# cipherflow-fhe/lattisense

Measured on AMD Instinct MI355X. Metric: ckks_hmult_relin_rescale_throughput, higher is better.
Workload: dtype u64

## Files before the change

include/lattisense_amd.h:

```cpp
#ifndef LATTISENSE_AMD_H
#define LATTISENSE_AMD_H
#include <stddef.h>
#include <stdint.h>

#ifdef __cplusplus
extern "C" {
#endif

typedef struct lsa_context_st* lsa_context;
typedef struct lsa_key_st* lsa_key;

enum { LSA_OK = 0, LSA_ERR_ARG = 1, LSA_ERR_NO_DEVICE = 2, LSA_ERR_HIP = 3, LSA_ERR_INTERNAL = 4 };
enum { LSA_ALGO_BFV = 0, LSA_ALGO_CKKS = 1 };

const char* lsa_last_error(void);
const char* lsa_version(void);
const char* lsa_build_flags(void);

int lsa_context_create(int algo, int n, const uint64_t* q, int nq, const uint64_t* p, int np, uint64_t t,
                       int device, lsa_context* out);
int lsa_context_destroy(lsa_context ctx);
int lsa_context_moduli(lsa_context ctx, uint64_t* out, int capacity, int* count);

int lsa_malloc(lsa_context ctx, void** dptr, size_t bytes);
// ... 70 lines not shown
                          const uint64_t* const* pts, const long long* spts, const uint64_t* partial, long long spartial,
                          uint64_t* out, int batch, long long sout, void* stream);
int lsa_bfv_rotate_mac_plain_mul(lsa_context ctx, int level, const uint64_t* in, int n, const uint64_t* galois_elements,
                                 const lsa_key* glk, const uint64_t* const* pts, const long long* spts, const uint64_t* partial,
                                 long long spartial, uint64_t* out, int batch, long long sin, long long sout, void* stream);
int lsa_bfv_rescale(lsa_context ctx, int level, int polys, const uint64_t* in, uint64_t* out, int batch,
                    long long stride_in, long long stride_out, void* stream);
int lsa_bfv_mult_relin(lsa_context ctx, int level, const uint64_t* a, const uint64_t* b, lsa_key rlk,
                       uint64_t* out, int batch, long long stride_a, long long stride_b, long long stride_out,
                       void* stream);

int lsa_set_tile_batch(lsa_context ctx, int tile_batch);
int lsa_set_fp64_ntt(lsa_context ctx, int enable);
int lsa_set_dual_stream(lsa_context ctx, int enable);
int lsa_set_fuse_tails(lsa_context ctx, int enable);
int lsa_set_ntt_chunk_mib(lsa_context ctx, int mib);
int lsa_ckks_rotate_many(lsa_context ctx, int level, const uint64_t* in, int n_rot, const uint64_t* galois_elements,
                         const lsa_key* glk, uint64_t* const* outs, int batch, long long sin, long long sout, void* stream);
int lsa_bfv_rotate_many(lsa_context ctx, int level, const uint64_t* in, int n_rot, const uint64_t* galois_elements,
                        const lsa_key* glk, uint64_t* const* outs, int batch, long long sin, long long sout, void* stream);

typedef struct lsa_bootstrap_st* lsa_bootstrap;
int lsa_bootstrap_create(lsa_context ctx, int cts_depth, int stc_depth, int k, int double_angle, double message_ratio,
                         double in_scale, double out_scale, int log_slots, void* stream, lsa_bootstrap* out);
int lsa_bootstrap_create_ex(lsa_context ctx, int cts_depth, int stc_depth, int k, int double_angle, double message_ratio,
                            double in_scale, double out_scale, int log_slots, int sine_deg, int arcsine_deg, void* stream,
                            lsa_bootstrap* out);
int lsa_bootstrap_evalmod_constants(lsa_bootstrap b, int* n_cheb, double* cheb, int* n_asin, double* asin_coef);
void lsa_bootstrap_destroy(lsa_bootstrap b);
int lsa_bootstrap_info(lsa_bootstrap b, int* out_level, double* out_scale, int* n_galois, int* n_matrices, int* n_cts,
// ... 54 lines not shown
```

lattisense_amd/_native.py:

```python
import ctypes
import importlib.util
import os

_HERE = os.path.dirname(os.path.abspath(__file__))
LIB_PATH = os.environ.get("LSA_NATIVE_LIB") or os.path.join(_HERE, "liblattisense_amd.so")

_lib = None

c_u64p = ctypes.POINTER(ctypes.c_uint64)
c_ll = ctypes.c_longlong
c_vp = ctypes.c_void_p
c_int = ctypes.c_int


class LsaError(RuntimeError):
    def __init__(self, code, msg):
        super().__init__("lattisense_amd error %d: %s" % (code, msg))
        self.code = code


def _preload_hip_runtime():
    spec = importlib.util.find_spec("torch")
    if spec is not None and spec.origin:
        p = os.path.join(os.path.dirname(spec.origin), "lib", "libamdhip64.so")
# ... 46 lines not shown
    "lsa_ckks_mult_const": (c_int, [c_vp, c_int, c_vp, c_ll, ctypes.c_double, ctypes.c_double, ctypes.c_double, c_vp, c_ll, c_int,
                                    c_int, c_vp]),
    "lsa_ckks_add_const": (c_int, [c_vp, c_int, c_vp, c_ll, ctypes.c_double, ctypes.c_double, ctypes.c_double, c_vp, c_ll, c_int,
                                   c_vp]),
    "lsa_ckks_affine_const": (c_int, [c_vp, c_int, c_vp, c_ll, ctypes.c_double, ctypes.c_double, ctypes.c_double, ctypes.c_double,
                                      ctypes.c_double, ctypes.c_double, c_vp, c_ll, c_int, c_int, c_vp]),
    "lsa_bfv_mult": (c_int, [c_vp, c_int, c_vp, c_vp, c_vp, c_int, c_ll, c_ll, c_ll, c_vp]),
    "lsa_bfv_relin": (c_int, [c_vp, c_int, c_vp, c_vp, c_vp, c_int, c_ll, c_ll, c_vp]),
    "lsa_bfv_rotate": (c_int, [c_vp, c_int, c_vp, ctypes.c_uint64, c_vp, c_vp, c_int, c_ll, c_ll, c_vp]),
    "lsa_bfv_rescale": (c_int, [c_vp, c_int, c_int, c_vp, c_vp, c_int, c_ll, c_ll, c_vp]),
    "lsa_bfv_mult_relin": (c_int, [c_vp, c_int, c_vp, c_vp, c_vp, c_vp, c_int, c_ll, c_ll, c_ll, c_vp]),
    "lsa_set_tile_batch": (c_int, [c_vp, c_int]),
    "lsa_set_fp64_ntt": (c_int, [c_vp, c_int]),
    "lsa_set_dual_stream": (c_int, [c_vp, c_int]),
    "lsa_set_fuse_tails": (c_int, [c_vp, c_int]),
    "lsa_set_ntt_chunk_mib": (c_int, [c_vp, c_int]),
    "lsa_debug_set_ntt_stamps": (c_int, [c_vp, c_vp]),
    "lsa_debug_baseconv_plans": (c_int, [c_vp, c_int, ctypes.POINTER(c_int), ctypes.POINTER(c_int), ctypes.POINTER(c_int),
                                         ctypes.POINTER(c_int)]),
    "lsa_debug_key_switch_fused": (c_int, [c_vp, c_int, c_vp, ctypes.POINTER(c_int)]),
    "lsa_ckks_rotate_many": (c_int, [c_vp, c_int, c_vp, c_int, c_u64p, ctypes.POINTER(c_vp), ctypes.POINTER(c_vp), c_int,
                                     ctypes.c_longlong, ctypes.c_longlong, c_vp]),
    "lsa_bfv_rotate_many": (c_int, [c_vp, c_int, c_vp, c_int, c_u64p, ctypes.POINTER(c_vp), ctypes.POINTER(c_vp), c_int,
                                    ctypes.c_longlong, ctypes.c_longlong, c_vp]),
    "lsa_bfv_mult_plain_mul": (c_int, [c_vp, c_int, c_vp, c_vp, c_vp, c_int, c_ll, c_ll, c_ll, c_vp]),
    "lsa_bfv_mac_plain_mul": (c_int, [c_vp, c_int, c_int, ctypes.POINTER(c_vp), ctypes.POINTER(c_ll), ctypes.POINTER(c_vp),
                                      ctypes.POINTER(c_ll), c_vp, c_ll, c_vp, c_int, c_ll, c_vp]),
    "lsa_bfv_rotate_mac_plain_mul": (c_int, [c_vp, c_int, c_vp, c_int, c_u64p, ctypes.POINTER(c_vp), ctypes.POINTER(c_vp),
                                             ctypes.POINTER(c_ll), c_vp, c_ll, c_vp, c_int, c_ll, c_ll, c_vp]),
    "lsa_bootstrap_create": (c_int, [c_vp, c_int, c_int, c_int, c_int, ctypes.c_double, ctypes.c_double, ctypes.c_double, c_int,
# ... 77 lines not shown
```

lattisense_amd/csrc/build_flags.h:

```cpp
#pragma once

#if (defined(LSA_NTT_DIAG_NO_TWIDDLE_LOADS) || defined(LSA_NTT_DIAG_COPY_ONLY) || defined(LSA_NTT_DIAG_COMPUTE_ONLY) || defined(LSA_NTT_DIAG_TW8) || \
     defined(LSA_KS_DIAG_NO_MATH) || defined(LSA_KS_DIAG_NO_STORE) || defined(LSA_BC_DIAG_NO_MATH) || defined(LSA_BC_DIAG_NO_STORE)) && \
    !defined(LSA_DIAG_BUILD)
#error "wrong-result diagnostic switches need -DLSA_DIAG_BUILD (use lattisense_amd.build --variant: it adds the flag and renames the library)"
#endif

#define LSA_BF_STR2(x) #x
#define LSA_BF_STR(x) LSA_BF_STR2(x)

#define LSA_BUILD_FLAGS_TEXT_1 ""
#ifdef LSA_DIAG_BUILD
#define LSA_BF_DIAG " LSA_DIAG_BUILD"
#else
#define LSA_BF_DIAG ""
#endif
#ifdef LSA_NTT_DIAG_NO_TWIDDLE_LOADS
#define LSA_BF_A " LSA_NTT_DIAG_NO_TWIDDLE_LOADS"
#else
#define LSA_BF_A ""
#endif
#ifdef LSA_NTT_DIAG_COPY_ONLY
#define LSA_BF_B " LSA_NTT_DIAG_COPY_ONLY"
#else
// ... 127 lines not shown
#if defined(LSA_KSMAC_WAVES_FP) && LSA_KSMAC_WAVES_FP != 2
#define LSA_BF_AE " LSA_KSMAC_WAVES_FP=" LSA_BF_STR(LSA_KSMAC_WAVES_FP)
#else
#define LSA_BF_AE ""
#endif
#if defined(LSA_KSMAC_CHUNK) && LSA_KSMAC_CHUNK != 4
#define LSA_BF_AF " LSA_KSMAC_CHUNK=" LSA_BF_STR(LSA_KSMAC_CHUNK)
#else
#define LSA_BF_AF ""
#endif
#ifdef LSA_NTT_DIAG_TW8
#define LSA_BF_AD " LSA_NTT_DIAG_TW8"
#else
#define LSA_BF_AD ""
#endif
#ifdef LSA_VARIANT_NAME
#define LSA_BF_V " variant=" LSA_BF_STR(LSA_VARIANT_NAME)
#else
#define LSA_BF_V ""
#endif
#ifdef LSA_AB_SWITCH
#define LSA_BF_W " LSA_AB_SWITCH=" LSA_BF_STR(LSA_AB_SWITCH)
#else
#define LSA_BF_W ""
#endif

#define LSA_BUILD_FLAGS_TEXT                                                                                              \
    LSA_BF_DIAG LSA_BF_A LSA_BF_B LSA_BF_C LSA_BF_D LSA_BF_E LSA_BF_F LSA_BF_G LSA_BF_H LSA_BF_I LSA_BF_J LSA_BF_K LSA_BF_L \
        LSA_BF_M LSA_BF_N LSA_BF_O LSA_BF_P LSA_BF_Q LSA_BF_R LSA_BF_S LSA_BF_T LSA_BF_U LSA_BF_V LSA_BF_W LSA_BF_X LSA_BF_Y LSA_BF_Z LSA_BF_AA LSA_BF_AB LSA_BF_AC LSA_BF_AD LSA_BF_AE LSA_BF_AF
```

lattisense_amd/csrc/c_api.hip:

```cpp
#include "build_flags.h"
#include "linear_transform.h"
#include "poly_eval.h"
#include "lsa_internal.h"

namespace lsa {
const char* kernels_build_flags();
const char* context_build_flags();
}

using namespace lsa;

struct lsa_context_st {
    Context ctx;
    lsa_context_st(int algo, int n, const u64* q, int nq, const u64* p, int np, u64 t, int dev)
        : ctx(algo, n, q, nq, p, np, t, dev) {}
};
struct lsa_key_st {
    Key key;
    double* fp_owned = nullptr;
};

template <typename F>
static int guard(F&& f) {
    try {
// ... 354 lines not shown

int lsa_profile_read_primary(lsa_context ctx, int kind, double* total_bytes_primary) {
    return guard([&] {
        Context& c = C(ctx);
        LSA_REQUIRE(kind >= 0 && kind < LSA_PROF_KINDS && total_bytes_primary, "bad argument");
        double by = 0;
        for (auto& sm : c.prof_samples)
            if (sm.kid == kind) by += sm.bytes_primary;
        *total_bytes_primary = by;
    });
}

int lsa_set_fuse_tails(lsa_context ctx, int enable) {
    return guard([&] { C(ctx).fuse_tails = enable ? 1 : 0; });
}
int lsa_set_dual_stream(lsa_context ctx, int enable) {
    return guard([&] { C(ctx).dual_stream = enable ? 1 : 0; });
}
int lsa_debug_set_ntt_stamps(lsa_context ctx, void* device_buffer) {
    return guard([&] { C(ctx).ntt_diag = static_cast<unsigned long long*>(device_buffer); });
}
int lsa_debug_baseconv_plans(lsa_context ctx, int capacity, int* count, int* ns, int* nd, int* split) {
    return guard([&] {
        Context& c = C(ctx);
        LSA_REQUIRE(count != nullptr && (capacity == 0 || (ns && nd && split)), "null argument");
        std::lock_guard<std::mutex> lk(c.mu);
        *count = (int)c.bconv.size();
        int i = 0;
        for (auto& kv : c.bconv) {
            if (i >= capacity) break;
// ... 382 lines not shown
```

lattisense_amd/csrc/emu_ntt.cpp:

```cpp
#define LSA_EMULATE 1
#include <cstddef>
#include <vector>
#include "ntt_plan.h"
#include "ntt_r16.h"
#include <array>
#include "tables.h"

template <int NT>
static void emu_block(const NttPassArgs& a, const NttBlockCtx& bc, u64* lds) {
    for (int t = 0; t < NT; t++) ntt_phase_load<true, NT, true>(a, bc, t, lds);
    int rho[4];
    const int np = ntt_split(a.mu, rho);
    if (!a.inverse) {
        int sig = 0;
        for (int i = 0; i < np; i++) {
            for (int t = 0; t < NT; t++) ntt_phase_sub_dyn<NT>(a, bc, t, lds, sig, rho[i]);
            sig += rho[i];
        }
    } else {
        int sig = a.mu;
        for (int i = np - 1; i >= 0; i--) {
            sig -= rho[i];
            for (int t = 0; t < NT; t++) ntt_phase_sub_dyn<NT>(a, bc, t, lds, sig, rho[i]);
        }
    }
    for (int t = 0; t < NT; t++) ntt_phase_store<true, NT>(a, bc, t, lds);
}

template <int PASS, int MU>
static void emu_block_r16(const NttPassArgs& a, const NttBlockCtx& bc, u64* lds) {
    std::vector<std::array<u64, 16>> regs(LSA_R16_THREADS);
    for (int phase = 0; phase < 3; phase++)
        for (int t = 0; t < LSA_R16_THREADS; t++) {
            u64(&v)[16] = *reinterpret_cast<u64(*)[16]>(regs[t].data());
            r16_phase<PASS, 3 | 16, MU>(a, bc, t, lds, phase, v);
        }
}

static void emu_block_r8x3(const NttPassArgs& a, const NttBlockCtx& bc, u64* lds) {
    std::vector<std::array<u64, 16>> regs(LSA_R16_THREADS);
    for (int phase = 0; phase < 4; phase++)
        for (int t = 0; t < LSA_R16_THREADS; t++) {
            u64(&v)[16] = *reinterpret_cast<u64(*)[16]>(regs[t].data());
            r8x3_phase<3 | 16>(a, bc, t, lds, phase, v);
        }
}

static int emu_ntt(int n, const u64* moduli, int nmod, u64* data, int batch, long long batch_stride, int rows,
                   const unsigned char* mod_of, int period, int inverse, int tau_max, int allow_fp64, const u64* pa, const u64* pb) {
    const int row_inner = (allow_fp64 >> 1) & 1;
    const bool r16 = (allow_fp64 >> 2) & 1;
    allow_fp64 &= 1;
    lsa::HostTables T;
    T.build(n, std::vector<u64>(moduli, moduli + nmod));
    NttPlan plan = make_ntt_plan(T.logn, tau_max);
    std::vector<u64> tw_i(T.psi.size());
    std::vector<double> tw_d(T.psi_d.size());
    for (int m = 0; m < nmod; m++) {
        const size_t o = (size_t)m * n;
        ntt_permute_twiddles(plan, T.logn, (inverse ? T.psiinv : T.psi).data() + 2 * o, tw_i.data() + 2 * o, 2, false);
        ntt_permute_twiddles(plan, T.logn, (inverse ? T.psiinv_d : T.psi_d).data() + o, tw_d.data() + o, 1, true);
    }
    NttPassArgs a{};
    a.src = data;
// ... 9 lines not shown
    a.scaled = T.scale_d.data();
    a.allow_fp64 = allow_fp64;
    a.period = period;
    a.row0 = 0;
    a.row_step = 1;
    a.row_inner = row_inner;
    for (int i = 0; i < period; i++) a.mod_of[i] = mod_of[i];
    if (pa) {
        a.fz_pro = 3;
        a.fz_limbs = rows;
        a.fz_a = pa;
        a.fz_b = pb;
        a.fz_a_stride = a.fz_b_stride = batch_stride;
        a.fz_a_rpp = a.fz_b_rpp = rows;
    }
    int launch_rows = 0;
    for (int r = 0; r < rows; r++)
        if (mod_of[r % period] != LSA_ROW_SKIP) a.row_tbl[launch_rows++] = (unsigned short)r;
    a.compact = 1;
    a.rows = launch_rows;
    for (int step = 0; step < plan.npass; step++) {
        int k = inverse ? plan.npass - 1 - step : step;
        ntt_fill_pass(a, plan, T.logn, k, inverse);
        a.fz_first = step == 0;
        a.fp_raw_out = plan.npass == 2 && step == 0;
        a.fp_raw_in = plan.npass == 2 && step == 1;
        std::vector<u64> lds(lds_words(a.tau));
        long long nblocks = (long long)batch * launch_rows * (1 << (a.logn - a.tau));
        for (long long bid = 0; bid < nblocks; bid++) {
            NttBlockCtx bc = ntt_decode_block(a, bid);
            if (bc.mod == LSA_ROW_SKIP) continue;
            if (r16 && ntt_r16_shape_ok(a, plan.npass)) {
                if (a.mu == 9) emu_block_r8x3(a, bc, lds.data());
                else if (a.lambda && a.mu == 8) emu_block_r16<0, 8>(a, bc, lds.data());
                else if (a.lambda) emu_block_r16<0, 7>(a, bc, lds.data());
                else if (a.mu == 8) emu_block_r16<1, 8>(a, bc, lds.data());
                else emu_block_r16<1, 7>(a, bc, lds.data());
            } else if (a.tau <= 12) emu_block<LSA_NTT_THREADS>(a, bc, lds.data());
            else if (a.tau == 13) emu_block<512>(a, bc, lds.data());
            else emu_block<1024>(a, bc, lds.data());
        }
    }
    return 0;
}

extern "C" int lsa_emu_ntt(int n, const u64* moduli, int nmod, u64* data, int batch, long long batch_stride, int rows,
                           const unsigned char* mod_of, int period, int inverse, int tau_max, int allow_fp64) {
    return emu_ntt(n, moduli, nmod, data, batch, batch_stride, rows, mod_of, period, inverse, tau_max, allow_fp64, nullptr, nullptr);
}

extern "C" int lsa_emu_intt_prod(int n, const u64* moduli, int nmod, const u64* pa, const u64* pb, u64* out, int batch,
                                 long long batch_stride, int rows, const unsigned char* mod_of, int period, int tau_max,
                                 int allow_fp64) {
    if (!pa || !pb) return -1;
    return emu_ntt(n, moduli, nmod, out, batch, batch_stride, rows, mod_of, period, 1, tau_max, allow_fp64, pa, pb);
}
```

lattisense_amd/csrc/kernels.hip:

```cpp
#include <atomic>
#include <cstdlib>

#include "build_flags.h"
#include "lsa_internal.h"
#include "ntt_r16.h"
#include "plain_ops.h"
#include "poly_lincomb.h"
#include "tensor_sum.h"

namespace lsa {

const char* kernels_build_flags() { return LSA_BUILD_FLAGS_TEXT; }

static constexpr int TPB = 256;

#ifndef LSA_NTT_WAVES
#define LSA_NTT_WAVES 4
#endif

#if defined(LSA_NTT_DIAG_STAMPS)
#define LSA_STAMP(k)                                                                               \
    do {                                                                                           \
        if (a.diag && threadIdx.x == 0 && blockIdx.x < 8192) a.diag[blockIdx.x * 8 + (k)] = __builtin_amdgcn_s_memtime(); \
    } while (0)
// ... 127 lines not shown
    const bool pro = fused && a.fz_pro && a.fz_first, epi = fused && a.fz_epi && a.final_reduce;
    if (pro && a.fz_pro == 3) return 16;
    if (epi && a.fz_epi == 3) return 4;
    if (epi && a.fz_epi == 4) return 8;
    return (pro ? 1 : 0) | (epi ? 2 : 0);
}
template <int FZ>
static auto ntt_r16_second_pass(int mu) {
    return mu == 9 ? &k_ntt_r8x3<FZ> : mu == 8 ? &k_ntt_r16<1, FZ, 8> : &k_ntt_r16<1, FZ, 7>;
}
static bool ntt_launch_r16(const NttPassArgs& a, int npass, bool fused, long long nblocks, hipStream_t s) {
    if (!sw::ntt_r16() || !ntt_r16_shape_ok(a, npass)) return false;
    const int fz = ntt_pass_fz(a, fused);
    void (*k)(NttPassArgs) = nullptr;
    if (a.lambda) {
        if (fz == 1 && a.mu == 8 && sw::r16_pro()) k = &k_ntt_r16<0, 1, 8>;
        else if (fz == 0) k = a.mu == 8 ? &k_ntt_r16<0, 0, 8> : &k_ntt_r16<0, 0, 7>;
    } else if (a.mu != 9 || sw::ntt_r8x3()) {
        switch (fz) {
            case 0: k = ntt_r16_second_pass<0>(a.mu); break;
            case 2: k = ntt_r16_second_pass<2>(a.mu); break;
            case 4: k = ntt_r16_second_pass<4>(a.mu); break;
            case 8: k = ntt_r16_second_pass<8>(a.mu); break;
            case 16: k = a.inverse ? ntt_r16_second_pass<16>(a.mu) : nullptr; break;
        }
    }
    if (!k) return false;
    hipLaunchKernelGGL(k, dim3((unsigned)nblocks), dim3(LSA_R16_THREADS), (size_t)LSA_R16_LDS_WORDS * sizeof(u64), s, a);
    LSA_HIP(hipGetLastError());
    return true;
}
// ... 211 lines not shown
                const RowMap& rm, bool inverse, hipStream_t s, const NttFusion* fz, int passes) {
    if (batch <= 0 || rows <= 0) return;
    LSA_REQUIRE(rm.period >= 1 && rm.period <= LSA_MAX_PERIOD, "ntt: bad row-map period");
    NttPassArgs a{};
    a.batch = batch;
    a.rows = rows;
    a.mods = c.d_mods;
    a.scale = c.d_scale;
    a.diag = c.ntt_diag;
    a.scaled = c.d_scale_d;
    a.allow_fp64 = c.fp64_ntt;
    if (fz) {
        LSA_REQUIRE(!inverse || (fz->pro == 3 && !fz->epi), "inverse transforms take the product prologue only");
        LSA_REQUIRE(fz->pro != 3 || (inverse && !fz->epi && fz->a && fz->b && fz->limbs >= 1 && (passes & 1)),
                    "product prologue: an inverse transform from its first pass, two operands, no epilogue");
        a.fz_epi = fz->epi;
        a.fz_pro = fz->pro;
        a.fz_limbs = fz->limbs;
        a.fz_base_polys = fz->base_polys;
        a.fz_ql_mod = fz->ql_mod;
        a.fz_a = fz->a;
        a.fz_a_stride = fz->a_stride;
        a.fz_a_rpp = fz->a_rpp;
        a.fz_base = fz->base;
        a.fz_base_stride = fz->base_stride;
        a.fz_base_rpp = fz->base_rpp;
        a.fz_k = fz->k;
        a.fz_out = fz->out;
        a.fz_out_stride = fz->out_stride;
        a.fz_out_rpp = fz->out_rpp;
// ... 50 lines not shown
    if (passes != 3) wide = false;
    if (fz && fz->pro == 3) wide = false;
    const NttPlan& plan = wide ? c.plan_wide : c.plan;
    a.tw = wide ? (inverse ? c.d_psiinv_w : c.d_psi_w) : (inverse ? c.d_psiinv : c.d_psi);
    a.twd = wide ? (inverse ? c.d_psiinv_d_w : c.d_psi_d_w) : (inverse ? c.d_psiinv_d : c.d_psi_d);
    {
        bool any_fp = false, any_int = false;
        for (int r = 0; r < rows; r++) {
            const unsigned char m = rm.mod_of[(rm.row0 + r * rm.row_step) % rm.period];
            if (m == LSA_ROW_SKIP) continue;
            const bool fp = c.fp_engine(m);
            any_fp |= fp;
            any_int |= !fp;
        }
        a.row_inner = any_fp && any_int;
    }
    int chunk = batch;
    if (plan.npass > 1 && c.ntt_chunk_mib > 0) {
        const double per_item = 8.0 * c.n * std::max(active_rows, 1);
        chunk = (int)std::max(1.0, std::min((double)batch, c.ntt_chunk_mib * 1048576.0 / per_item));
    }
    for (int b0 = 0; b0 < batch; b0 += chunk) {
        const int nb = std::min(chunk, batch - b0);
        a.batch = nb;
        if (fz && fz->epi == 3) {
            a.fz_a = fz->a + (long long)b0 * fz->a_stride;
            a.fz_base = fz->base ? fz->base + (long long)b0 * fz->base_stride : nullptr;
            a.fz_out = fz->out + (long long)b0 * fz->out_stride;
        }
        if (fz && fz->epi == 4) {
            a.fz_a = fz->a + (long long)b0 * fz->a_stride;
            a.fz_base = fz->base ? fz->base + (long long)b0 * fz->base_stride : nullptr;
            a.fz_pt = fz->pt + (long long)b0 * fz->pt_stride;
            a.fz_out = fz->out + (long long)b0 * fz->out_stride;
        }
        if (fz && fz->pro == 3) {
            a.fz_a = fz->a + (long long)b0 * fz->a_stride;
            a.fz_b = fz->b + (long long)b0 * fz->b_stride;
        }
        bool first = true;
        for (int step = 0; step < plan.npass; step++) {
            if (plan.npass == 2 && !((passes >> step) & 1)) continue;
            a.fz_first = first ? 1 : 0;
            first = false;
            const int k = inverse ? plan.npass - 1 - step : step;
            ntt_fill_pass(a, plan, c.logn, k, inverse ? 1 : 0);
            a.fp_raw_out = plan.npass == 2 && step == 0 && c.fp_raw;
            a.fp_raw_in = plan.npass == 2 && step == 1 && c.fp_raw;
            LSA_REQUIRE(!(a.fz_first && a.fz_pro && a.fp_raw_in), "ntt: a fused prologue reads canonical inputs, never a raw hand-off");
            a.src = (step == 0 ? src + (long long)b0 * src_stride : dst + (long long)b0 * dst_stride);
// ... 1929 lines not shown
```

lattisense_amd/csrc/lsa_internal.h:

```cpp
#pragma once
#include <hip/hip_runtime.h>
#include <cstdint>
#include <map>
#include <memory>
#include <mutex>
#include <stdexcept>
#include <string>
#include <vector>

#include "../../include/lattisense_amd.h"
#include "ntt_plan.h"
#include "plain_ops.h"
#include "switches.h"
#include "tables.h"

namespace lsa {

struct Error : std::runtime_error {
    int code;
    Error(int c, const std::string& m) : std::runtime_error(m), code(c) {}
};

void set_last_error(const std::string& m);

// ... 57 lines not shown
    int wide_mode = 2;
    ModDev* d_mods = nullptr;
    u64* d_psi = nullptr;
    u64* d_psiinv = nullptr;
    u64* d_scale = nullptr;
    double* d_psi_d = nullptr;
    double* d_psiinv_d = nullptr;
    u64* d_psi_w = nullptr;
    u64* d_psiinv_w = nullptr;
    double* d_psi_d_w = nullptr;
    double* d_psiinv_d_w = nullptr;
    double* d_scale_d = nullptr;
    int fp64_ntt = 1;
    int tile_batch = 0;
    int fp_raw = 1;
    int fuse_tails = 1;
    int dual_stream = 0;
    hipStream_t aux_stream = nullptr;
    hipEvent_t ev_fork = nullptr, ev_join = nullptr;
    void fork_aux(hipStream_t s);
    void join_aux(hipStream_t s);
    unsigned long long* ntt_diag = nullptr;
    int ntt_chunk_mib = 0;

    struct ProfSample {
        hipEvent_t e0, e1;
        int kid;
        double bytes;
        double bytes_primary;
    };
// ... 300 lines not shown
```

lattisense_amd/csrc/ntt_core.h:

```cpp
#pragma once
#include "modarith.h"

#ifndef LSA_NTT_THREADS
#define LSA_NTT_THREADS 256
#endif
#define LSA_MAX_PERIOD 192
#if defined(LSA_EMULATE)
#include <cstdio>
#include <cstdlib>
#define LSA_EMU_CHECK(c) do { if (!(c)) { std::fprintf(stderr, "ntt replay: range invariant violated: %s (%s:%d)\n", #c, __FILE__, __LINE__); std::abort(); } } while (0)
#else
#define LSA_EMU_CHECK(c) do { } while (0)
#endif
#define LSA_ROW_SKIP 0xFF
#define LSA_FP64_MAX_BITS 47
#ifndef LSA_NTT_MAX_RHO
#define LSA_NTT_MAX_RHO 4
#endif

struct NttPassArgs {
    const u64* src;
    u64* dst;
    long long src_stride;
    long long dst_stride;
// ... 212 lines not shown
LSA_HD u64 double_to_u52(double r) { return d_to_bits(r + 4503599627370496.0) & 0x000FFFFFFFFFFFFFull; }
LSA_HD double fp_modmul(double v, double w, double q, double qinv) {
    const double h = v * w;
    const double l = __builtin_fma(v, w, -h);
    const double c = __builtin_rint(h * qinv);
    const double d = __builtin_fma(-c, q, h);
    return d + l;
}
LSA_HD double fp_reduce(double x, double q, double qinv) { return __builtin_fma(-__builtin_rint(x * qinv), q, x); }

#define LSA_NTT_STAGE_PAIRS 8
#ifndef LSA_NTT_HEAD_ROUNDS
#define LSA_NTT_HEAD_ROUNDS 2
#endif
struct NttLoadFix {
    bool head, add, fp, near, raw, fp_lift;
    u64 ql, h, hq;
    double hd, qld;
    ModDev mi;
};
LSA_HD u64 ntt_load_fix(const NttLoadFix& f, u64 v, u64 t) {
    if (f.fp_lift) {
        const double td = u52_to_double(t);
        const double r = td > f.hd ? td - f.qld : td;
        return d_to_bits(f.add ? u52_to_double(v) + r : r);
    }
    if (f.head) {
        const u64 c = add_mod(t, f.h, f.ql);
        const u64 lift = sub_mod(f.near ? csub(c, f.mi.q) : reduce_u64(c, f.mi), f.hq, f.mi.q);
        v = f.add ? add_mod(v, lift, f.mi.q) : lift;
    }
    if (f.fp && !f.raw) v = d_to_bits(u52_to_double(v));
    return v;
}
template <bool FZ>
LSA_HD NttLoadFix ntt_make_load_fix(const NttPassArgs& a, const NttBlockCtx& bc, const u64*& g, const u64*& gl) {
    g = a.src + bc.base_src;
    gl = g;
    NttLoadFix f;
    f.head = FZ && (a.fz_pro == 1 || a.fz_pro == 2) && a.fz_first;
    f.add = f.head && a.fz_pro == 2;
    f.fp = bc.fp != 0;
    f.raw = f.fp && a.fp_raw_in;
    LSA_EMU_CHECK(!(a.fz_pro && a.fz_first && a.fp_raw_in));
    f.mi = a.mods[bc.mod];
    f.ql = f.h = f.hq = 0;
    f.hd = f.qld = 0.0;
    f.near = f.fp_lift = false;
    if (f.head) {
        gl = a.fz_last + (long long)bc.b * a.fz_last_stride + ((long long)(bc.row / a.fz_limbs) * a.fz_last_rpp << a.logn);
        if (!f.add) g = gl;
        f.ql = a.mods[a.fz_ql_mod].q;
        f.h = (f.ql - 1) >> 1;
        f.hq = reduce_u64(f.h, f.mi);
        f.near = f.ql <= 2 * f.mi.q;
        f.fp_lift = f.fp && (f.ql >> 48) == 0;
        f.hd = (double)f.h;
        f.qld = (double)f.ql;
    }
    return f;
}
struct NttProdFix {
    const u64* pa;
// ... 52 lines not shown
            lds[lds_addr(2 * i)] = ntt_prod_fix(pf, pf.pa[x], pf.pb[x]);
            lds[lds_addr(2 * i + 1)] = ntt_prod_fix(pf, pf.pa[x + 1], pf.pb[x + 1]);
        }
        return;
    }
    const NttLoadFix f = ntt_make_load_fix<FZ>(a, bc, g, gl);
    const NttTileMap tm = ntt_tile_map(a, bc.tile);
    if (half == LSA_NTT_STAGE_PAIRS * NT && !f.add) {
        NttLoadFix f1 = f;
        f1.add = false;
        u64 st[2 * LSA_NTT_STAGE_PAIRS];
#pragma unroll
        for (int p = 0; p < LSA_NTT_STAGE_PAIRS; p++) {
            const int x = ntt_tile_index(tm, 2 * (tid + p * NT));
            ntt_load_data_pair(g + x, st[2 * p], st[2 * p + 1]);
        }
#pragma unroll
        for (int p = 0; p < LSA_NTT_STAGE_PAIRS; p++) {
            const int l = 2 * (tid + p * NT);
            lds[lds_addr(l)] = ntt_load_fix(f1, st[2 * p], st[2 * p]);
            lds[lds_addr(l + 1)] = ntt_load_fix(f1, st[2 * p + 1], st[2 * p + 1]);
        }
        return;
    }
    if (half == LSA_NTT_STAGE_PAIRS * NT) {
        constexpr int CH = LSA_NTT_STAGE_PAIRS / LSA_NTT_HEAD_ROUNDS;
#pragma unroll 1
        for (int p0 = 0; p0 < LSA_NTT_STAGE_PAIRS; p0 += CH) {
            u64 st[2 * CH], sl[2 * CH];
#pragma unroll
// ... 635 lines not shown
```

lattisense_amd/csrc/ntt_r16.h:

```cpp
#pragma once
#include "ntt_core.h"

#define LSA_R16_THREADS 256
#define LSA_R16_LDS_WORDS (272 * 16)

LSA_HD bool ntt_r16_shape_ok(const NttPassArgs& a, int npass) {
    if (npass != 2 || a.tau != 12) return false;
    if (a.mu == 9) return a.s_lo == a.logn - 9 && a.lambda == 0;
    if (a.mu != 8 && a.mu != 7) return false;
    return (a.s_lo == 0 && a.lambda == 12 - a.mu) || (a.s_lo == a.logn - a.mu && a.lambda == 0);
}

template <int PASS, int MU>
LSA_HD int r16_lds(int k, int i) {
    const int p = i + (i >> 4);
    return PASS == 0 ? (p << (12 - MU)) + k : k * ((1 << MU) + (1 << (MU - 4))) + p;
}
template <int PASS, int MU>
LSA_HD long long r16_x(const NttPassArgs& a, int tile, int k, int i) {
    return PASS == 0 ? ((long long)tile << (12 - MU)) + ((long long)i << (a.logn - MU)) + k : ((long long)tile << 12) + (k << MU) + i;
}
template <int MU, int IMAGE>
LSA_HD int r16_pt(int i, int e) {
    return IMAGE == 0 ? i + (e << (MU - 4)) : 16 * i + e;
// ... 67 lines not shown
LSA_HD void r16_lane(int tid, int& k, int& i) {
    if (PASS == 0) {
        k = tid & ((1 << (12 - MU)) - 1);
        i = tid >> (12 - MU);
    } else {
        i = tid & ((1 << (MU - 4)) - 1);
        k = tid >> (MU - 4);
    }
}
template <int PASS, int MU>
LSA_HD unsigned r16_G1(const NttBlockCtx& bc, int k) {
    return PASS == 0 ? 0u : ((unsigned)bc.tile << (12 - MU)) + (unsigned)k;
}


template <int PASS, bool FZ, int IMAGE, int MU>
LSA_HD void r16_load_direct(const NttPassArgs& a, const NttBlockCtx& bc, int tid, u64 (&v)[16]) {
    const u64* g;
    const u64* gl;
    const NttLoadFix f = ntt_make_load_fix<FZ>(a, bc, g, gl);
    int k, i;
    r16_lane<PASS, MU>(tid, k, i);
    u64 t[16];
    if (FZ && f.add) {
#pragma unroll
        for (int h = 0; h < 2; h++) {
#pragma unroll
            for (int e = 8 * h; e < 8 * h + 8; e++) {
                const long long x = r16_x<PASS, MU>(a, bc.tile, k, r16_pt<MU, IMAGE>(i, e));
                v[e] = r16_load1(g + x);
                t[e] = r16_load1(gl + x);
            }
            if (f.fp_lift) {
#pragma unroll
                for (int e = 8 * h; e < 8 * h + 8; e++) {
                    const double td = u52_to_double(t[e]);
                    const double r = td > f.hd ? td - f.qld : td;
                    v[e] = d_to_bits(u52_to_double(v[e]) + r);
                }
            } else {
#pragma unroll
                for (int e = 8 * h; e < 8 * h + 8; e++) v[e] = ntt_load_fix(f, v[e], t[e]);
            }
        }
        return;
    }
#pragma unroll
    for (int e = 0; e < 16; e++) v[e] = r16_load1(g + r16_x<PASS, MU>(a, bc.tile, k, r16_pt<MU, IMAGE>(i, e)));
    if (!(FZ && f.head)) {
        if (f.fp && !f.raw) {
#pragma unroll
            for (int e = 0; e < 16; e++) v[e] = d_to_bits(u52_to_double(v[e]));
        }
        return;
    }
    NttLoadFix f1 = f;
    f1.add = false;
#pragma unroll
    for (int e = 0; e < 16; e++) v[e] = ntt_load_fix(f1, v[e], v[e]);
}
template <int PASS, bool FZ, int IMAGE, int MU>
LSA_HD void r16_store_direct(const NttPassArgs& a, const NttBlockCtx& bc, int tid, const u64 (&v)[16]) {
    u64* g;
    const u64* pa;
// ... 274 lines not shown
            r16_dpp_stage<1>(d, L.twd, L.s_lo, G1, i, L.q, L.qinv);
            r16_dpp_stage<2>(d, L.twd, L.s_lo, G1, i, L.q, L.qinv);
            r16_dpp_stage<3>(d, L.twd, L.s_lo, G1, i, L.q, L.qinv);
#pragma unroll
            for (int e = 0; e < 16; e++) v[e] = d_to_bits(d[e]);
            r16_group<PASS, 1, MU>(v, a, bc, L, G2);
            r16_lds_put<PASS, 1, MU>(tid, lds, v);
        } else {
            r16_store_coalesced<(FZ & 2) != 0, MU, (FZ & 4) != 0, (FZ & 8) != 0>(a, bc, tid, lds);
        }
        return;
    }
#endif
    if (!a.inverse) {
        if (phase == 0) {
            r16_load_direct<PASS, (FZ & 1) != 0, 0, MU>(a, bc, tid, v);
            r16_group<PASS, 0, MU>(v, a, bc, L, G1);
            r16_lds_put<PASS, 0, MU>(tid, lds, v);
        } else if (phase == 1) {
            r16_lds_get<PASS, 1, MU>(tid, lds, v);
            r16_group<PASS, 1, MU>(v, a, bc, L, G2);
            if (PASS == 0) r16_store_direct<PASS, (FZ & 2) != 0, 1, MU>(a, bc, tid, v);
            else r16_lds_put<PASS, 1, MU>(tid, lds, v);
        } else if (PASS == 1) {
            r16_store_coalesced<(FZ & 2) != 0, MU, (FZ & 4) != 0, (FZ & 8) != 0>(a, bc, tid, lds);
        }
    } else {
        if (phase == 0) {
            if (PASS == 0) r16_load_direct<PASS, false, 1, MU>(a, bc, tid, v);
            else r16_load_coalesced<false, MU, (FZ & 16) != 0>(a, bc, tid, lds);
        } else if (phase == 1) {
// ... 250 lines not shown
```

lattisense_amd/csrc/ops.hip:

```cpp
#include "layout_check.h"
#include "linear_transform.h"
#include "lsa_internal.h"
#include "plain_ops.h"
#include "tensor_sum.h"

namespace lsa {

static RowMap rm_seq(int count, int first = 0) {
    RowMap r;
    LSA_REQUIRE(count >= 1 && count <= LSA_MAX_PERIOD, "row map too long");
    r.period = count;
    for (int i = 0; i < count; i++) r.mod_of[i] = (unsigned char)(first + i);
    return r;
}

static int ceil_div(int a, int b) { return (a + b - 1) / b; }

struct KsRescale {
    u64* out;
    long long sout;
};

struct RotMacTerm {
    const u64* pt;
// ... 176 lines not shown
            NttFusion fz;
            fz.pro = 3;
            fz.limbs = L;
            fz.a = prod->a + prod->pa;
            fz.a_stride = prod->sa;
            fz.a_rpp = (int)(prod->pa >> c.logn);
            fz.b = prod->b + prod->pb;
            fz.b_stride = prod->sb;
            fz.b_rpp = (int)(prod->pb >> c.logn);
            launch_ntt(c, cxi, cxi, nb, s_cxi, s_cxi, L, rm_seq(L), true, s, &fz);
        } else if (!cx_coef) {
            launch_ntt(c, cx, cxi, nb, scx, s_cxi, L, rm_seq(L), true, s);
        }
        const u64* conv_src = cx_coef ? cx_coef : cxi;
        const long long s_src = cx_coef ? s_coef : s_cxi;
        for (int d = 0; d < beta; d++) {
            const int d0 = d * np, d1 = std::min(d0 + np, L);
            std::vector<int> src, dst;
            BaseConvRows rows{};
            for (int i = d0; i < d1; i++) {
                rows.src_row[i - d0] = i;
                src.push_back(i);
            }
            for (int tl = 0; tl < T; tl++) {
                if (tl >= d0 && tl < d1) continue;
                rows.dst_row[dst.size()] = d * T + tl;
                dst.push_back(c.qp_mod(L, tl));
            }
            launch_baseconv(c, c.baseconv(src, dst, false), rows, conv_src, ext, nb, s_src, s_ext, s);
        }
        auto own = [&](int d, int tl) { return tl >= d * np && tl < std::min((d + 1) * np, L); };
        if (beta * T <= LSA_MAX_PERIOD) {
            RowMap rm;
            rm.period = beta * T;
            for (int d = 0; d < beta; d++)
                for (int tl = 0; tl < T; tl++) rm.mod_of[d * T + tl] = own(d, tl) ? LSA_ROW_SKIP : (unsigned char)c.qp_mod(L, tl);
            launch_ntt(c, ext, ext, nb, s_ext, s_ext, beta * T, rm, false, s, nullptr, fused ? 1 : 3);
            if (!fused) return;
            bool any = false;
            for (int i = 0; i < beta * T; i++) {
                if (rm.mod_of[i] == LSA_ROW_SKIP) continue;
                if (ks_fused_limb(c, L, i % T)) rm.mod_of[i] = LSA_ROW_SKIP;
                else any = true;
            }
            if (any) launch_ntt(c, ext, ext, nb, s_ext, s_ext, beta * T, rm, false, s, nullptr, 2);
            return;
        }
        for (int d = 0; d < beta; d++) {
            RowMap rm;
            rm.period = T;
            for (int tl = 0; tl < T; tl++) rm.mod_of[tl] = own(d, tl) ? LSA_ROW_SKIP : (unsigned char)c.qp_mod(L, tl);
            launch_ntt(c, ext + (size_t)d * T * N, ext + (size_t)d * T * N, nb, s_ext, s_ext, T, rm, false, s);
        }
    }

    void mac(const u64* cx, long long scx, const Key& k, const TensorFold* fold = nullptr) {
        if (!fused) {
            launch_ks_mac(c, level, cx, scx, ext, s_ext, k, acc, s_acc, nb, s, false, nullptr, nullptr, 0, fold);
            return;
        }
        LSA_REQUIRE(&k == key, "fused key MAC: the tile was planned for another key");
        LSA_REQUIRE(launch_ntt_ksmac(c, level, cx, scx, ext, s_ext, k, acc, s_acc, nb, s, fold), "fused key MAC: shape not covered");
        launch_ks_mac(c, level, cx, scx, ext, s_ext, k, acc, s_acc, nb, s, true, nullptr, nullptr, 0, fold);
    }

    void moddown(const KsOut& o) { ks_moddown(c, level, acc, s_acc, conv, o, nb, s); }
};
// ... 1047 lines not shown
```

lattisense_amd/device.py:

```python
import ctypes

import numpy as np

from . import _native
from ._native import check, lib

ALGO_BFV, ALGO_CKKS = 0, 1


class DeviceBuffer:
    def __init__(self, ctx, nwords):
        self.ctx = ctx
        self.nwords = int(nwords)
        p = ctypes.c_void_p()
        check(lib().lsa_malloc(ctx.h, ctypes.byref(p), self.nwords * 8))
        self.ptr = p.value

    def free(self):
        if self.ptr:
            check(lib().lsa_free(self.ctx.h, self.ptr))
            self.ptr = None

    def __del__(self):
        try:
# ... 50 lines not shown
    def set_tile_batch(self, tb):
        check(lib().lsa_set_tile_batch(self.h, tb))

    def baseconv_plans(self):
        cnt = ctypes.c_int()
        check(lib().lsa_debug_baseconv_plans(self.h, 0, ctypes.byref(cnt), None, None, None))
        n = cnt.value
        ns, nd, sp = (ctypes.c_int * max(n, 1))(), (ctypes.c_int * max(n, 1))(), (ctypes.c_int * max(n, 1))()
        check(lib().lsa_debug_baseconv_plans(self.h, n, ctypes.byref(cnt), ns, nd, sp))
        return [(ns[i], nd[i], bool(sp[i])) for i in range(min(n, cnt.value))]

    def key_switch_fused(self, level, key):
        out = ctypes.c_int()
        check(lib().lsa_debug_key_switch_fused(self.h, level, key, ctypes.byref(out)))
        return bool(out.value)

    def set_fp64_ntt(self, enable):
        check(lib().lsa_set_fp64_ntt(self.h, int(enable)))

    def upload_key(self, compact, key_level):
        compact = np.ascontiguousarray(compact, dtype=np.uint64)
        assert compact.nbytes == lib().lsa_key_bytes(self.h, key_level), "key shape does not match its level"
        k = ctypes.c_void_p()
        check(lib().lsa_key_upload(self.h, compact.ctypes.data, key_level, self.stream, ctypes.byref(k)))
        return k

    def adopt_key(self, dev_ptr, key_level):
        k = ctypes.c_void_p()
        check(lib().lsa_key_adopt_device(self.h, dev_ptr, key_level, self.stream, ctypes.byref(k)))
        return k
# ... 447 lines not shown
```

Baseline: 14270.

## Fuse single-limb modup base conversion into the forward NTT load as a lift prologue

When a key-switch decomposition digit holds a single limb with a modulus below 2^53, the base-conversion kernel is skipped for it. The reduction of that source limb into each extended modulus is done inside the forward NTT's first-pass load through a new lift prologue (fz_pro=4), in both the radix-16 and staged paths. This removes one kernel launch and a write/read round trip of the extended rows for such digits. The cost is an extra NTT launch that splits rows into lifted and converted groups, a forced row-inner ordering, and more kernel template variants. It is enabled by default through a new context flag.

```diff
diff --git a/include/lattisense_amd.h b/include/lattisense_amd.h
--- a/include/lattisense_amd.h
+++ b/include/lattisense_amd.h
@@ -108,6 +108,7 @@
 int lsa_set_fp64_ntt(lsa_context ctx, int enable);
 int lsa_set_dual_stream(lsa_context ctx, int enable);
 int lsa_set_fuse_tails(lsa_context ctx, int enable);
+int lsa_set_modup_lift(lsa_context ctx, int enable);
 int lsa_set_ntt_chunk_mib(lsa_context ctx, int mib);
 int lsa_ckks_rotate_many(lsa_context ctx, int level, const uint64_t* in, int n_rot, const uint64_t* galois_elements,
                          const lsa_key* glk, uint64_t* const* outs, int batch, long long sin, long long sout, void* stream);
diff --git a/lattisense_amd/_native.py b/lattisense_amd/_native.py
--- a/lattisense_amd/_native.py
+++ b/lattisense_amd/_native.py
@@ -84,6 +84,7 @@
     "lsa_set_fp64_ntt": (c_int, [c_vp, c_int]),
     "lsa_set_dual_stream": (c_int, [c_vp, c_int]),
     "lsa_set_fuse_tails": (c_int, [c_vp, c_int]),
+    "lsa_set_modup_lift": (c_int, [c_vp, c_int]),
     "lsa_set_ntt_chunk_mib": (c_int, [c_vp, c_int]),
     "lsa_debug_set_ntt_stamps": (c_int, [c_vp, c_vp]),
     "lsa_debug_baseconv_plans": (c_int, [c_vp, c_int, ctypes.POINTER(c_int), ctypes.POINTER(c_int), ctypes.POINTER(c_int),
diff --git a/lattisense_amd/csrc/build_flags.h b/lattisense_amd/csrc/build_flags.h
--- a/lattisense_amd/csrc/build_flags.h
+++ b/lattisense_amd/csrc/build_flags.h
@@ -165,6 +165,11 @@
 #else
 #define LSA_BF_AD ""
 #endif
+#ifdef LSA_LIFT_ROW_OUTER
+#define LSA_BF_AG " LSA_LIFT_ROW_OUTER"
+#else
+#define LSA_BF_AG ""
+#endif
 #ifdef LSA_VARIANT_NAME
 #define LSA_BF_V " variant=" LSA_BF_STR(LSA_VARIANT_NAME)
 #else
@@ -178,4 +183,4 @@
 
 #define LSA_BUILD_FLAGS_TEXT                                                                                              \
     LSA_BF_DIAG LSA_BF_A LSA_BF_B LSA_BF_C LSA_BF_D LSA_BF_E LSA_BF_F LSA_BF_G LSA_BF_H LSA_BF_I LSA_BF_J LSA_BF_K LSA_BF_L \
-        LSA_BF_M LSA_BF_N LSA_BF_O LSA_BF_P LSA_BF_Q LSA_BF_R LSA_BF_S LSA_BF_T LSA_BF_U LSA_BF_V LSA_BF_W LSA_BF_X LSA_BF_Y LSA_BF_Z LSA_BF_AA LSA_BF_AB LSA_BF_AC LSA_BF_AD LSA_BF_AE LSA_BF_AF
+        LSA_BF_M LSA_BF_N LSA_BF_O LSA_BF_P LSA_BF_Q LSA_BF_R LSA_BF_S LSA_BF_T LSA_BF_U LSA_BF_V LSA_BF_W LSA_BF_X LSA_BF_Y LSA_BF_Z LSA_BF_AA LSA_BF_AB LSA_BF_AC LSA_BF_AD LSA_BF_AE LSA_BF_AF LSA_BF_AG
diff --git a/lattisense_amd/csrc/c_api.hip b/lattisense_amd/csrc/c_api.hip
--- a/lattisense_amd/csrc/c_api.hip
+++ b/lattisense_amd/csrc/c_api.hip
@@ -392,6 +392,9 @@
 int lsa_set_fuse_tails(lsa_context ctx, int enable) {
     return guard([&] { C(ctx).fuse_tails = enable ? 1 : 0; });
 }
+int lsa_set_modup_lift(lsa_context ctx, int enable) {
+    return guard([&] { C(ctx).modup_lift = enable ? 1 : 0; });
+}
 int lsa_set_dual_stream(lsa_context ctx, int enable) {
     return guard([&] { C(ctx).dual_stream = enable ? 1 : 0; });
 }
diff --git a/lattisense_amd/csrc/emu_ntt.cpp b/lattisense_amd/csrc/emu_ntt.cpp
--- a/lattisense_amd/csrc/emu_ntt.cpp
+++ b/lattisense_amd/csrc/emu_ntt.cpp
@@ -27,13 +27,13 @@
     for (int t = 0; t < NT; t++) ntt_phase_store<true, NT>(a, bc, t, lds);
 }
 
-template <int PASS, int MU>
+template <int PASS, int MU, int FZ = 3 | 16>
 static void emu_block_r16(const NttPassArgs& a, const NttBlockCtx& bc, u64* lds) {
     std::vector<std::array<u64, 16>> regs(LSA_R16_THREADS);
     for (int phase = 0; phase < 3; phase++)
         for (int t = 0; t < LSA_R16_THREADS; t++) {
             u64(&v)[16] = *reinterpret_cast<u64(*)[16]>(regs[t].data());
-            r16_phase<PASS, 3 | 16, MU>(a, bc, t, lds, phase, v);
+            r16_phase<PASS, FZ, MU>(a, bc, t, lds, phase, v);
         }
 }
 
@@ -47,7 +47,8 @@
 }
 
 static int emu_ntt(int n, const u64* moduli, int nmod, u64* data, int batch, long long batch_stride, int rows,
-                   const unsigned char* mod_of, int period, int inverse, int tau_max, int allow_fp64, const u64* pa, const u64* pb) {
+                   const unsigned char* mod_of, int period, int inverse, int tau_max, int allow_fp64, const u64* pa, const u64* pb,
+                   const u64* lift = nullptr, int lift_mod = 0, int lift_limbs = 1) {
     const int row_inner = (allow_fp64 >> 1) & 1;
     const bool r16 = (allow_fp64 >> 2) & 1;
     allow_fp64 &= 1;
@@ -87,6 +88,14 @@
         a.fz_a_stride = a.fz_b_stride = batch_stride;
         a.fz_a_rpp = a.fz_b_rpp = rows;
     }
+    if (lift) {
+        a.fz_pro = 4;
+        a.fz_limbs = lift_limbs;
+        a.fz_last = lift;
+        a.fz_last_stride = (long long)(rows / lift_limbs) * n;
+        a.fz_last_rpp = 1;
+        a.fz_ql_mod = lift_mod;
+    }
     int launch_rows = 0;
     for (int r = 0; r < rows; r++)
         if (mod_of[r % period] != LSA_ROW_SKIP) a.row_tbl[launch_rows++] = (unsigned short)r;
@@ -105,6 +114,7 @@
             if (bc.mod == LSA_ROW_SKIP) continue;
             if (r16 && ntt_r16_shape_ok(a, plan.npass)) {
                 if (a.mu == 9) emu_block_r8x3(a, bc, lds.data());
+                else if (a.lambda && lift) (a.mu == 8 ? emu_block_r16<0, 8, 32> : emu_block_r16<0, 7, 32>)(a, bc, lds.data());
                 else if (a.lambda && a.mu == 8) emu_block_r16<0, 8>(a, bc, lds.data());
                 else if (a.lambda) emu_block_r16<0, 7>(a, bc, lds.data());
                 else if (a.mu == 8) emu_block_r16<1, 8>(a, bc, lds.data());
@@ -128,3 +138,11 @@
     if (!pa || !pb) return -1;
     return emu_ntt(n, moduli, nmod, out, batch, batch_stride, rows, mod_of, period, 1, tau_max, allow_fp64, pa, pb);
 }
+
+extern "C" int lsa_emu_ntt_lift(int n, const u64* moduli, int nmod, const u64* src, int src_mod, int limbs, u64* out, int batch,
+                                long long batch_stride, int rows, const unsigned char* mod_of, int period, int tau_max,
+                                int allow_fp64) {
+    if (!src || limbs < 1 || rows % limbs || src_mod < 0 || src_mod + rows / limbs > nmod) return -1;
+    return emu_ntt(n, moduli, nmod, out, batch, batch_stride, rows, mod_of, period, 0, tau_max, allow_fp64, nullptr, nullptr, src,
+                   src_mod, limbs);
+}
diff --git a/lattisense_amd/csrc/kernels.hip b/lattisense_amd/csrc/kernels.hip
--- a/lattisense_amd/csrc/kernels.hip
+++ b/lattisense_amd/csrc/kernels.hip
@@ -165,7 +165,8 @@
     const int fz = ntt_pass_fz(a, fused);
     void (*k)(NttPassArgs) = nullptr;
     if (a.lambda) {
-        if (fz == 1 && a.mu == 8 && sw::r16_pro()) k = &k_ntt_r16<0, 1, 8>;
+        if (fz == 1 && a.fz_pro == 4 && sw::r16_pro()) k = a.mu == 8 ? &k_ntt_r16<0, 32, 8> : &k_ntt_r16<0, 32, 7>;
+        else if (fz == 1 && a.fz_pro != 4 && a.mu == 8 && sw::r16_pro()) k = &k_ntt_r16<0, 1, 8>;
         else if (fz == 0) k = a.mu == 8 ? &k_ntt_r16<0, 0, 8> : &k_ntt_r16<0, 0, 7>;
     } else if (a.mu != 9 || sw::ntt_r8x3()) {
         switch (fz) {
@@ -407,6 +408,8 @@
         LSA_REQUIRE(!inverse || (fz->pro == 3 && !fz->epi), "inverse transforms take the product prologue only");
         LSA_REQUIRE(fz->pro != 3 || (inverse && !fz->epi && fz->a && fz->b && fz->limbs >= 1 && (passes & 1)),
                     "product prologue: an inverse transform from its first pass, two operands, no epilogue");
+        LSA_REQUIRE(fz->pro != 4 || (!inverse && !fz->epi && fz->last && fz->limbs >= 1 && (passes & 1)),
+                    "lift prologue: a forward transform from its first pass, one source row per polynomial, no epilogue");
         a.fz_epi = fz->epi;
         a.fz_pro = fz->pro;
         a.fz_limbs = fz->limbs;
@@ -487,6 +490,11 @@
             any_int |= !fp;
         }
         a.row_inner = any_fp && any_int;
+#if defined(LSA_LIFT_ROW_OUTER)
+        if (fz && fz->pro == 4) a.row_inner = 0;
+#else
+        if (fz && fz->pro == 4) a.row_inner = 1;
+#endif
     }
     int chunk = batch;
     if (plan.npass > 1 && c.ntt_chunk_mib > 0) {
@@ -507,6 +515,7 @@
             a.fz_pt = fz->pt + (long long)b0 * fz->pt_stride;
             a.fz_out = fz->out + (long long)b0 * fz->out_stride;
         }
+        if (fz && fz->pro == 4) a.fz_last = fz->last + (long long)b0 * fz->last_stride;
         if (fz && fz->pro == 3) {
             a.fz_a = fz->a + (long long)b0 * fz->a_stride;
             a.fz_b = fz->b + (long long)b0 * fz->b_stride;
diff --git a/lattisense_amd/csrc/lsa_internal.h b/lattisense_amd/csrc/lsa_internal.h
--- a/lattisense_amd/csrc/lsa_internal.h
+++ b/lattisense_amd/csrc/lsa_internal.h
@@ -95,6 +95,7 @@
     int fp64_ntt = 1;
     int tile_batch = 0;
     int fp_raw = 1;
+    int modup_lift = 1;
     int fuse_tails = 1;
     int dual_stream = 0;
     hipStream_t aux_stream = nullptr;
diff --git a/lattisense_amd/csrc/ntt_core.h b/lattisense_amd/csrc/ntt_core.h
--- a/lattisense_amd/csrc/ntt_core.h
+++ b/lattisense_amd/csrc/ntt_core.h
@@ -250,12 +250,39 @@
 #define LSA_NTT_HEAD_ROUNDS 2
 #endif
 struct NttLoadFix {
-    bool head, add, fp, near, raw, fp_lift;
+    bool head, add, fp, near, raw, fp_lift, lift;
     u64 ql, h, hq;
     double hd, qld;
     ModDev mi;
 };
+template <int NE>
+LSA_HD void ntt_lift_block(const NttLoadFix& f, u64* v) {
+    if (f.fp_lift && f.near) {
+#pragma unroll
+        for (int e = 0; e < NE; e++) {
+            const double x = u52_to_double(v[e]);
+            v[e] = d_to_bits(x >= f.qld ? x - f.qld : x);
+        }
+    } else if (f.fp_lift) {
+#pragma unroll
+        for (int e = 0; e < NE; e++) v[e] = d_to_bits(fp_reduce(u52_to_double(v[e]), f.qld, f.hd));
+    } else if (f.near) {
+#pragma unroll
+        for (int e = 0; e < NE; e++) v[e] = csub(v[e], f.mi.q);
+    } else {
+#pragma unroll
+        for (int e = 0; e < NE; e++) v[e] = reduce_u64(v[e], f.mi);
+    }
+    if (f.fp && !f.fp_lift) {
+#pragma unroll
+        for (int e = 0; e < NE; e++) v[e] = d_to_bits(u52_to_double(v[e]));
+    }
+}
 LSA_HD u64 ntt_load_fix(const NttLoadFix& f, u64 v, u64 t) {
+    if (f.lift) {
+        ntt_lift_block<1>(f, &v);
+        return v;
+    }
     if (f.fp_lift) {
         const double td = u52_to_double(t);
         const double r = td > f.hd ? td - f.qld : td;
@@ -269,12 +296,12 @@
     if (f.fp && !f.raw) v = d_to_bits(u52_to_double(v));
     return v;
 }
-template <bool FZ>
+template <bool FZ, int LIFT = 1>
 LSA_HD NttLoadFix ntt_make_load_fix(const NttPassArgs& a, const NttBlockCtx& bc, const u64*& g, const u64*& gl) {
     g = a.src + bc.base_src;
     gl = g;
     NttLoadFix f;
-    f.head = FZ && (a.fz_pro == 1 || a.fz_pro == 2) && a.fz_first;
+    f.head = FZ && LIFT != 2 && (a.fz_pro == 1 || a.fz_pro == 2) && a.fz_first;
     f.add = f.head && a.fz_pro == 2;
     f.fp = bc.fp != 0;
     f.raw = f.fp && a.fp_raw_in;
@@ -283,6 +310,16 @@
     f.ql = f.h = f.hq = 0;
     f.hd = f.qld = 0.0;
     f.near = f.fp_lift = false;
+    f.lift = FZ && LIFT != 0 && a.fz_pro == 4 && a.fz_first;
+    if (f.lift) {
+        const int poly = bc.row / a.fz_limbs;
+        g = gl = a.fz_last + (long long)bc.b * a.fz_last_stride + ((long long)poly * a.fz_last_rpp << a.logn);
+        f.ql = a.mods[a.fz_ql_mod + poly * a.fz_last_rpp].q;
+        f.near = f.ql <= 2 * f.mi.q;
+        f.fp_lift = f.fp && (f.ql >> 52) == 0;
+        f.qld = (double)f.mi.q;
+        f.hd = 1.0 / f.qld;
+    }
     if (f.head) {
         gl = a.fz_last + (long long)bc.b * a.fz_last_stride + ((long long)(bc.row / a.fz_limbs) * a.fz_last_rpp << a.logn);
         if (!f.add) g = gl;
@@ -365,6 +402,16 @@
         for (int p = 0; p < LSA_NTT_STAGE_PAIRS; p++) {
             const int x = ntt_tile_index(tm, 2 * (tid + p * NT));
             ntt_load_data_pair(g + x, st[2 * p], st[2 * p + 1]);
+        }
+        if (FZ && f.lift) {
+            ntt_lift_block<2 * LSA_NTT_STAGE_PAIRS>(f, st);
+#pragma unroll
+            for (int p = 0; p < LSA_NTT_STAGE_PAIRS; p++) {
+                const int l = 2 * (tid + p * NT);
+                lds[lds_addr(l)] = st[2 * p];
+                lds[lds_addr(l + 1)] = st[2 * p + 1];
+            }
+            return;
         }
 #pragma unroll
         for (int p = 0; p < LSA_NTT_STAGE_PAIRS; p++) {
diff --git a/lattisense_amd/csrc/ntt_r16.h b/lattisense_amd/csrc/ntt_r16.h
--- a/lattisense_amd/csrc/ntt_r16.h
+++ b/lattisense_amd/csrc/ntt_r16.h
@@ -105,15 +105,15 @@
 }
 
 
-template <int PASS, bool FZ, int IMAGE, int MU>
+template <int PASS, bool FZ, int IMAGE, int MU, int LIFT = 0>
 LSA_HD void r16_load_direct(const NttPassArgs& a, const NttBlockCtx& bc, int tid, u64 (&v)[16]) {
     const u64* g;
     const u64* gl;
-    const NttLoadFix f = ntt_make_load_fix<FZ>(a, bc, g, gl);
+    const NttLoadFix f = ntt_make_load_fix<FZ, LIFT>(a, bc, g, gl);
     int k, i;
     r16_lane<PASS, MU>(tid, k, i);
     u64 t[16];
-    if (FZ && f.add) {
+    if (FZ && LIFT != 2 && f.add) {
 #pragma unroll
         for (int h = 0; h < 2; h++) {
 #pragma unroll
@@ -138,7 +138,11 @@
     }
 #pragma unroll
     for (int e = 0; e < 16; e++) v[e] = r16_load1(g + r16_x<PASS, MU>(a, bc.tile, k, r16_pt<MU, IMAGE>(i, e)));
-    if (!(FZ && f.head)) {
+    if (FZ && LIFT != 0 && f.lift) {
+        ntt_lift_block<16>(f, v);
+        return;
+    }
+    if (!(FZ && LIFT != 2 && f.head)) {
         if (f.fp && !f.raw) {
 #pragma unroll
             for (int e = 0; e < 16; e++) v[e] = d_to_bits(u52_to_double(v[e]));
@@ -443,7 +447,7 @@
 #endif
     if (!a.inverse) {
         if (phase == 0) {
-            r16_load_direct<PASS, (FZ & 1) != 0, 0, MU>(a, bc, tid, v);
+            r16_load_direct<PASS, (FZ & (1 | 32)) != 0, 0, MU, (FZ & 32) ? 2 : 0>(a, bc, tid, v);
             r16_group<PASS, 0, MU>(v, a, bc, L, G1);
             r16_lds_put<PASS, 0, MU>(tid, lds, v);
         } else if (phase == 1) {
diff --git a/lattisense_amd/csrc/ops.hip b/lattisense_amd/csrc/ops.hip
--- a/lattisense_amd/csrc/ops.hip
+++ b/lattisense_amd/csrc/ops.hip
@@ -214,7 +214,15 @@
         }
         const u64* conv_src = cx_coef ? cx_coef : cxi;
         const long long s_src = cx_coef ? s_coef : s_cxi;
+        const bool lift_on = c.modup_lift != 0;
+        auto lifted = [&](int d) { return lift_on && std::min(d * np + np, L) - d * np == 1 && (c.T.mods[d * np].q >> 53) == 0; };
+        bool any_lift = false, any_conv = false;
         for (int d = 0; d < beta; d++) {
+            if (lifted(d)) {
+                any_lift = true;
+                continue;
+            }
+            any_conv = true;
             const int d0 = d * np, d1 = std::min(d0 + np, L);
             std::vector<int> src, dst;
             BaseConvRows rows{};
@@ -230,18 +238,29 @@
             launch_baseconv(c, c.baseconv(src, dst, false), rows, conv_src, ext, nb, s_src, s_ext, s);
         }
         auto own = [&](int d, int tl) { return tl >= d * np && tl < std::min((d + 1) * np, L); };
+        NttFusion lf;
+        lf.pro = 4;
+        lf.limbs = T;
+        lf.last = conv_src;
+        lf.last_stride = s_src;
+        lf.last_rpp = np;
+        lf.ql_mod = 0;
         if (beta * T <= LSA_MAX_PERIOD) {
-            RowMap rm;
-            rm.period = beta * T;
+            RowMap rm, rl;
+            rm.period = rl.period = beta * T;
             for (int d = 0; d < beta; d++)
-                for (int tl = 0; tl < T; tl++) rm.mod_of[d * T + tl] = own(d, tl) ? LSA_ROW_SKIP : (unsigned char)c.qp_mod(L, tl);
-            launch_ntt(c, ext, ext, nb, s_ext, s_ext, beta * T, rm, false, s, nullptr, fused ? 1 : 3);
+                for (int tl = 0; tl < T; tl++) {
+                    const unsigned char m = own(d, tl) ? LSA_ROW_SKIP : (unsigned char)c.qp_mod(L, tl);
+                    rm.mod_of[d * T + tl] = lifted(d) ? LSA_ROW_SKIP : m;
+                    rl.mod_of[d * T + tl] = lifted(d) ? m : LSA_ROW_SKIP;
+                }
+            if (any_conv) launch_ntt(c, ext, ext, nb, s_ext, s_ext, beta * T, rm, false, s, nullptr, fused ? 1 : 3);
+            if (any_lift) launch_ntt(c, ext, ext, nb, s_ext, s_ext, beta * T, rl, false, s, &lf, fused ? 1 : 3);
             if (!fused) return;
             bool any = false;
             for (int i = 0; i < beta * T; i++) {
-                if (rm.mod_of[i] == LSA_ROW_SKIP) continue;
-                if (ks_fused_limb(c, L, i % T)) rm.mod_of[i] = LSA_ROW_SKIP;
-                else any = true;
+                rm.mod_of[i] = own(i / T, i % T) || ks_fused_limb(c, L, i % T) ? LSA_ROW_SKIP : (unsigned char)c.qp_mod(L, i % T);
+                any |= rm.mod_of[i] != LSA_ROW_SKIP;
             }
             if (any) launch_ntt(c, ext, ext, nb, s_ext, s_ext, beta * T, rm, false, s, nullptr, 2);
             return;
@@ -250,7 +269,9 @@
             RowMap rm;
             rm.period = T;
             for (int tl = 0; tl < T; tl++) rm.mod_of[tl] = own(d, tl) ? LSA_ROW_SKIP : (unsigned char)c.qp_mod(L, tl);
-            launch_ntt(c, ext + (size_t)d * T * N, ext + (size_t)d * T * N, nb, s_ext, s_ext, T, rm, false, s);
+            lf.last = conv_src + (size_t)d * np * N;
+            lf.ql_mod = d * np;
+            launch_ntt(c, ext + (size_t)d * T * N, ext + (size_t)d * T * N, nb, s_ext, s_ext, T, rm, false, s, lifted(d) ? &lf : nullptr);
         }
     }
 
diff --git a/lattisense_amd/device.py b/lattisense_amd/device.py
--- a/lattisense_amd/device.py
+++ b/lattisense_amd/device.py
@@ -88,6 +88,9 @@
         out = ctypes.c_int()
         check(lib().lsa_debug_key_switch_fused(self.h, level, key, ctypes.byref(out)))
         return bool(out.value)
+
+    def set_modup_lift(self, enable):
+        check(lib().lsa_set_modup_lift(self.h, int(enable)))
 
     def set_fp64_ntt(self, enable):
         check(lib().lsa_set_fp64_ntt(self.h, int(enable)))
```

Result: faster. 14740 (median of 6 runs) (+3.3%).
